# lighttransport/pbrlab

Measured on AMD Instinct MI355X. Metric: Msamples/s (paths x spp / s), 1920x1080 Cornell-box-Suzanne render, higher is better.
Workload: dtype f32

## Files before the change

pbrlab_amd/csrc/kernels.hip:

```cpp
#include <type_traits>

#include "dcamera.h"
#include "dshade.h"
#include "kernels.h"
#include "dtrace_pv.h"
#include "dtrace_quad.h"

namespace pb {

constexpr int kBlock = 256;

__device__ __forceinline__ uint32_t wave_sum(uint32_t v) {
#pragma unroll
  for (int o = 32; o > 0; o >>= 1) v += (uint32_t)__shfl_xor((int)v, o);
  return v;
}

__device__ __forceinline__ float4 mk4(V3 v, float w) { return make_float4(v.x, v.y, v.z, w); }

__device__ __forceinline__ void camera_sample(const PathState& P, uint32_t j, V3& dir, uint64_t& rng_state) {
  const uint32_t R = P.pass_run, q = j / R;
  const uint32_t pass = P.first_pass + (q / P.npix) * R + j % R;
  const uint32_t gpix = P.pix_index[q % P.npix];
  const uint32_t x = gpix % P.width, y = gpix / P.width;
// ... 442 lines not shown
      uint32_t i = tile * kTileItems + j * kBlock + threadIdx.x;
      e[j] = 0;
      if (i < n) e[j] = (i < n0) ? P.q_principled[i] : ((i < n0 + n1) ? P.q_hair[i - n0] : P.q_sss[i - n0 - n1]);
    }
    auto resumes = [](uint32_t w) { return (w & (kRAlive | kRResume)) == kRResume; };
    auto holds = [](uint32_t w) { return (w & (kRAlive | kRResume | kRHold)) == kRHold; };
    TileCompactor<2, kItemsPerThread> ta = {wcount, base, {}};
    {
      uint32_t dest[kItemsPerThread];
#pragma unroll
      for (int j = 0; j < kItemsPerThread; j++) dest[j] = ((e[j] & kRAlive) || resumes(e[j]) || holds(e[j])) ? 1u : 0u;
      ta.run(dest, counters);
#pragma unroll
      for (int j = 0; j < kItemsPerThread; j++)
        if (dest[j])
          P.q_out[ta.slot(j, 1u)] = resumes(e[j]) ? ((e[j] & (kRPathMask | kQDoomed)) | kQResume | ((e[j] & kRResumeFirst) ? kQFirst : 0u))
                                    : (holds(e[j]) ? ((e[j] & kRPathMask) | kQHold | ((e[j] & kRHoldDoomed) ? kQDoomed : 0u))
                                                   : (e[j] & (kRPathMask | kQSssBit | kQDoomed)));
      __syncthreads();
    }
    {
      uint32_t dest[kItemsPerThread];
#pragma unroll
      for (int j = 0; j < kItemsPerThread; j++) dest[j] = ((e[j] & kRShadow) && !resumes(e[j]) && !holds(e[j])) ? 2u : 0u;
      ta.run(dest, counters);
#pragma unroll
      for (int j = 0; j < kItemsPerThread; j++)
        if (dest[j]) P.q_shadow[ta.slot(j, 2u)] = e[j] & kRPathMask;
      __syncthreads();
    }
  }
}

struct PathHead {
  Hit h;
  V3 dir, thr;
  Surface s;
  Rng rng;
  uint32_t flags;
};
enum : int { kHeadEnds = 0, kHeadGoes = 1, kHeadHeld = 2 };
template <bool HOLD = true, bool ENV = false>
__device__ __forceinline__ int path_head(const PathState& P, const DScene& sc, uint32_t p, uint64_t rng_inc, PathHead& c, bool first) {
  float4 h4 = P.hit[p];
  float4 o4 = make_float4(P.cam_org[0], P.cam_org[1], P.cam_org[2], 0.0f), t4 = make_float4(1.0f, 1.0f, 1.0f, 0.0f);
  c.flags = first ? 0u : kFlagNotFirst;
  uint64_t rng_state;
  bool held = false;
  if (!first) {
    o4 = P.ray_o[p], t4 = P.thr[p];
    c.dir = ld3(P.ray_d[p]);
    if (HOLD) {
      const uint4 r4 = P.rng4[p];
      rng_state = (uint64_t)r4.x | ((uint64_t)r4.y << 32);
      held = P.no_medium != 0u && r4.z != 0u;
    } else {
      rng_state = P.rng[p];
    }
  } else {
    camera_sample(P, p - P.slot0, c.dir, rng_state);
  }
  c.h.t = h4.x, c.h.u = h4.y, c.h.v = h4.z, c.h.slot = __float_as_uint(h4.w);
  c.s = make_surface(sc, ld3(o4), c.dir, c.h);
  c.thr = ld3(t4);
  if (!held && c.s.face == kFront && c.s.lightrec != kNone) {
    const float4* lr = reinterpret_cast<const float4*>(sc.lrecs + c.s.lightrec);
    float pdf_area = lr[0].w;
    if (ENV) pdf_area = pdf_area * sc.env_area_scale;
    V3 emission = ld3(lr[4]);
    float a2s = fabsf((c.h.t * c.h.t) / dot(c.s.n_s, c.dir));
    float w = (c.flags & kFlagNotFirst) ? power_heuristic(t4.w, pdf_area * a2s) : 1.0f;
    float4 L4 = P.L[p];
    P.L[p] = mk4(ld3(L4) + w * emission * c.thr, L4.w);
  }
  c.rng.state = rng_state, c.rng.inc = rng_inc;
  float rr = spectrum_norm(c.thr);
  float u = draw(c.rng);
// ... 43 lines not shown
__device__ __forceinline__ bool misses_all_lights(const DScene& sc, V3 o, V3 d, float tmin) {
  if (sc.lights_transformed) return false;
  if (sc.num_lrecs <= kLightPretest) {
    const V3 inv(1.0f / d.x, 1.0f / d.y, 1.0f / d.z);
    for (uint32_t i = 0; i < sc.num_lrecs; i += 2u) {
      const float4* la = reinterpret_cast<const float4*>(sc.lrecs + i);
      const float4* lb = reinterpret_cast<const float4*>(sc.lrecs + (i + 1u < sc.num_lrecs ? i + 1u : i));
      const float4 a0 = la[0], a1 = la[1], a2 = la[2], b0 = lb[0], b1 = lb[1], b2 = lb[2];
      bool ok_a, ok_b;
      f2 t, u, v;
      tri_test_pair(make_float4(a0.x, b0.x, a0.y, b0.y), make_float4(a0.z, b0.z, a1.x, b1.x), make_float4(a1.y, b1.y, a1.z, b1.z),
                    make_float4(a2.x, b2.x, a2.y, b2.y), make_float4(a2.z, b2.z, 0.f, 0.f), o.x, o.y, o.z, d.x, d.y, d.z, inv.x, inv.y, inv.z, tmin, ok_a,
                    ok_b, t, u, v);
      if (ok_a || ok_b) return false;
    }
    return true;
  }
  if (sc.num_lights > kLightPretest) return false;
  const V3 inv(1.0f / d.x, 1.0f / d.y, 1.0f / d.z);
  for (uint32_t i = 0; i < (sc.num_lights + 1u) / 2u; i++) {
    const float4* np = reinterpret_cast<const float4*>(sc.light_boxes + i);
    bool h0, h1;
    float t0, t1;
    box_test2(np[0], np[1], np[2], o, inv, tmin, kInf, h0, h1, t0, t1);
    if (h0 || h1) return false;
  }
  return true;
}

__device__ __forceinline__ void count_pruned(const PathState& P) {
  if (P.stats) atomicAdd(&P.stats[kStatPrunedRays], 1ull);
}

__device__ __forceinline__ void put_shadow(const PathState& P, V3 pos, const Nee& n, V3 c_vis, V3 c_occ, uint32_t p,
                                           uint32_t mode, bool alive) {
  static_assert(kEps == 1e-3f, "shadow rays share (origin, tmin) with the continuation ray");
  if (!alive) P.ray_o[p] = mk4(pos, kEps);
  P.sh_d[p] = mk4(n.dir, smax(kEps, n.dist - kEps));
  P.sh_c[p] = mk4(c_vis, __uint_as_float(mode));
  if (mode == kShSssExit) P.sh_e[p] = mk4(c_occ, 0.f);
}

__device__ __forceinline__ bool stage_light_tables(const DScene& sc, float* lds) {
  if (!(sc.num_lights > 0 && sc.num_lights <= kLdsLights && sc.num_lrecs <= kLdsLights)) return false;
  constexpr uint32_t kRecWords = sizeof(LightRec) / 4;
  for (uint32_t i = threadIdx.x; i < sc.num_lights; i += kBlock) {
    lds[i] = sc.light_cdf[i];
    lds[kLdsLights + 2u * i] = __uint_as_float(sc.light_heads[i].first);
    lds[kLdsLights + 2u * i + 1u] = __uint_as_float(sc.light_heads[i].count);
  }
  for (uint32_t i = threadIdx.x; i < sc.num_lrecs; i += kBlock) lds[3u * kLdsLights + i] = sc.lprim_cdf[i];
  for (uint32_t i = threadIdx.x; i < sc.num_lrecs * kRecWords; i += kBlock) lds[4u * kLdsLights + i] = reinterpret_cast<const float*>(sc.lrecs)[i];
  return true;
}

enum : int { kShadePlain = 0, kShadeMedia = 1, kShadeFull = 2, kShadeEnv = 4 };
constexpr int shade_base(int mode) { return mode & 3; }
constexpr bool shade_env(int mode) { return (mode & kShadeEnv) != 0; }
template <int MODE_ = kShadeFull>
__device__ __forceinline__ uint32_t shade_principled_path(const PathState& P, const DScene& sc, uint32_t p, uint64_t rng_inc, bool first,
                                                          const PrincipledBsdf* lds_bsdf = nullptr, const float* lds_lights = nullptr) {
  constexpr int MODE = shade_base(MODE_);
  constexpr bool ENV = shade_env(MODE_);
  if (ENV && __float_as_uint(P.hit[p].w) == kNone) return env_miss_path<MODE != kShadeMedia>(P, sc, p, first);
  bool alive = false, shadow = false;
  V3 sh_pos(0.f), c_vis(0.f);
  Nee nee;
  nee.dir = V3(0.f), nee.emission = V3(0.f), nee.dist = 0.f, nee.pdf_sigma = 0.f;
  uint32_t sh_mode = kShNormal, qbit = 0u;
  PathHead c;
  const int head = path_head<MODE != kShadeMedia, ENV>(P, sc, p, rng_inc, c, first);
  if (head == kHeadGoes) {
    const Hit& h = c.h;
    const V3 dir = c.dir, thr = c.thr;
    const Surface& s = c.s;
    Rng& rng = c.rng;
    V3 new_thr(0.f), next_dir = -dir;
    float new_pdf = 0.f;
    if (s.face != kAmbiguous) {
      V3 wo_g = -dir;
      Frame fr;
      fr.ez = (s.face == kFront) ? s.n_s : -s.n_s;
      branchless_onb(fr.ez, fr.ex, fr.ey);
      V3 wo = to_local(fr, wo_g);
      PrincipledBsdf b;
      if (lds_bsdf) {
        constexpr uint32_t kWords = sizeof(PrincipledBsdf) / 4;
        const auto* lw = (const __attribute__((address_space(3))) uint32_t*)reinterpret_cast<const uint32_t*>(lds_bsdf) + s.material * kWords;
        uint32_t w[kWords];
#pragma unroll
        for (uint32_t k = 0; k < kWords; k++) w[k] = lw[k];
        __builtin_memcpy(&b, w, sizeof(b));
      } else {
        b = sc.materials[s.material].bsdf;
      }
      const bool per_hit = MODE == kShadeFull && sc.materials[s.material].textured != 0u;
      if (per_hit) {
        const PrincipledParam mp = sc.materials[s.material].param;
        V3 bc(mp.base_color[0], mp.base_color[1], mp.base_color[2]);
        V3 ssc(mp.subsurface_color[0], mp.subsurface_color[1], mp.subsurface_color[2]);
        if (mp.base_color_tex_id != kNone) bc = texture_fetch3(sc, mp.base_color_tex_id, s.tu, s.tv);
        if (mp.subsurface_color_tex_id != kNone) ssc = texture_fetch3(sc, mp.subsurface_color_tex_id, s.tu, s.tv);
        b = param_to_bsdf(mp, bc, ssc);
      }
// ... 23 lines not shown
      } else if (pick == 3) {
        float u0 = draw(rng);
        float u1 = draw(rng);
        ggx_sample(wo, b.clearcoat_alpha_x, b.clearcoat_alpha_y, u0, u1, wi);
      } else if (MODE == kShadePlain) {
        sampled = false;
      } else {
        sampled = false;
        bool ok = (s.face == kFront);
        if (ok) {
          float u0 = draw(rng);
          float u1 = draw(rng);
          V3 tmp;
          float pdf;
          lambert_sample(u0, u1, tmp, pdf);
          tmp = -tmp;
          V3 gdir = to_global(fr, tmp);
          ok = !(dot(-s.n_g, gdir) <= 0.0f);
          if (ok) {
            V3 sigt, sigs, wthr;
            if (per_hit) {
              medium_coefficients(b, sigt, sigs, wthr);
            } else {
              const float4* mc = reinterpret_cast<const float4*>(&sc.materials[s.material].sss_sigt);
              const float4 m0 = mc[0], m1 = mc[1], m2 = mc[2];
              sigt = V3(m0.x, m0.y, m0.z), sigs = V3(m0.w, m1.x, m1.y), wthr = V3(m1.z, m1.w, m2.x);
            }
            float e0 = draw(rng);
            float e1 = draw(rng);
            V3 chpdf;
            float t_scatter = sample_scatter_distance(wthr, sigs, sigt, e0, e1, chpdf);
            P.ray_o[p] = mk4(s.pos, 1e-3f);
            P.ray_d[p] = mk4(gdir, t_scatter);
            P.sss_sigt[p] = mk4(sigt, 0.f);
            P.sss_sigs[p] = mk4(sigs, __uint_as_float(sc.shade[h.slot & kHitSlotMask].instance_id));
            P.sss_thr[p] = mk4(wthr, __uint_as_float(0u));
            P.sss_ez[p] = mk4(fr.ez, 0.f);
            P.sss_A[p] = make_float4(0.f, 0.f, 0.f, 0.f);
            P.thr[p] = mk4(thr, 0.f);
            P.rng[p] = rng.state;
            alive = true;
            qbit = kQSssBit;
            sh_mode = kShSssEntry;
            c_vis = d1;
          }
        }
      }
      if (sampled) {
        V3 f;
        float pdf;
        eval_bsdf(wi, wo, b, w, f, pdf);
        next_dir = to_global(fr, wi);
        float cos_i = fabsf(wi.z);
        new_thr = f * cos_i / pdf;
        new_pdf = pdf;
        if (!is_finite(new_thr) || !isfinite(new_pdf)) {
          new_thr = V3(0.f);
          new_pdf = 0.f;
        }
      }
      if (sh_mode == kShNormal) c_vis = thr * ((V3(0.f) + d1) + V3(0.f));
      if (!alive) {
        V3 t2 = new_thr * thr;
        if (!is_black(t2)) {
          qbit = doomed_bit(t2, rng.state, rng_inc);
          if (!(qbit && !ENV && misses_all_lights(sc, s.pos, next_dir, 1e-3f))) {
            alive = true;
            P.ray_o[p] = mk4(s.pos, 1e-3f);
            P.ray_d[p] = mk4(next_dir, kInf);
            P.thr[p] = mk4(t2, new_pdf);
            store_rng<MODE != kShadeMedia>(P, p, rng.state);
          } else {
            qbit = 0u;
            count_pruned(P);
          }
        }
      }
    }
  }
  if (shadow) put_shadow(P, sh_pos, nee, c_vis, V3(0.f), p, sh_mode, alive);
  return head == kHeadHeld ? kRHold : ((shadow ? kRShadow : 0u) | (alive ? kRAlive : 0u) | qbit);
}
#ifndef PB_SHADE_WAVES
#define PB_SHADE_WAVES 4
#endif
#ifndef PB_LDS_MATS
#define PB_LDS_MATS 64
#endif
constexpr uint32_t kLdsMats = PB_LDS_MATS;
#ifndef PB_SHADE_WAVES_FULL
#define PB_SHADE_WAVES_FULL 3
#endif
#ifndef PB_SHADE_WAVES_MEDIA
#define PB_SHADE_WAVES_MEDIA 4
#endif
#ifndef PB_SHADE_WAVES_MEDIA_ENV
#define PB_SHADE_WAVES_MEDIA_ENV 3
#endif
constexpr int shade_waves(int mode) {
  return shade_base(mode) == kShadePlain ? PB_SHADE_WAVES
                                         : (shade_base(mode) == kShadeMedia ? (shade_env(mode) ? PB_SHADE_WAVES_MEDIA_ENV : PB_SHADE_WAVES_MEDIA) : PB_SHADE_WAVES_FULL);
}
template <int MODE_>
__global__ __launch_bounds__(kBlock, shade_waves(MODE_)) void k_shade_principled(PathState P, DScene sc, uint64_t rng_inc) {
  constexpr int MODE = shade_base(MODE_);
  constexpr bool ENV = shade_env(MODE_);
  __shared__ PrincipledBsdf lds_bsdf[kLdsMats ? kLdsMats : 1];
  __shared__ float lds_lights[kLdsMats ? kLdsLightWords : 1];
  const bool lights_staged = kLdsMats && stage_light_tables(sc, lds_lights);
  const bool staged = kLdsMats && sc.num_materials <= kLdsMats;
  if (staged) {
    constexpr uint32_t kWords = sizeof(PrincipledBsdf) / 4;
    static_assert(sizeof(PrincipledBsdf) % 4 == 0, "closure set is a whole number of words");
    uint32_t* dst = reinterpret_cast<uint32_t*>(lds_bsdf);
    for (uint32_t i = threadIdx.x; i < sc.num_materials * kWords; i += kBlock)
      dst[i] = reinterpret_cast<const uint32_t*>(&sc.materials[i / kWords].bsdf)[i % kWords];
  }
  if (staged || lights_staged) __syncthreads();
  const bool direct = P.direct != 0u;
  const uint32_t n = P.counts[direct ? kCntIn : kCntPrincipled];
  for (uint32_t i = blockIdx.x * kBlock + threadIdx.x; i < n; i += gridDim.x * kBlock) {
    constexpr bool kAnyBounce = MODE != kShadeMedia;
    const uint32_t e = direct ? ((!kAnyBounce || P.first) ? P.slot0 + i : P.q_in[i]) : P.q_principled[i];
    const uint32_t p = e & kQPathMask;
    uint32_t r = 0u;
    bool go = true;
    if (direct) {
      const uint32_t code = __float_as_uint(P.hit[p].w);
      const bool doomed = kAnyBounce && (e & kQDoomed);
      go = !(code == kNone || (!(code & kHitLight) && (doomed || (code & kHitNoMaterial))));
      if (ENV && code == kNone) go = true;
      if (code == kHitSuspended) {
        go = false, r = kRResume | kRResumeFirst;
        if (kAnyBounce && !P.first) r = kRResume | (e & kQDoomed) | ((e & kQFirst) ? kRResumeFirst : 0u);
      }
    } else if (e & kQResume) {
      go = false, r = kRResume | (e & kQDoomed) | ((e & kQFirst) ? kRResumeFirst : 0u);
    }
    if (go) r = shade_principled_path<MODE_>(P, sc, p, rng_inc, P.first != 0u || (e & kQFirst) != 0u, staged ? lds_bsdf : nullptr, lights_staged ? lds_lights : nullptr);
    if (r == kRHold && (e & kQDoomed) && (kAnyBounce ? !P.first : !direct)) r |= kRHoldDoomed;
    P.q_principled[i] = p | r;
  }
}

template <bool ENV = false>
__device__ __forceinline__ uint32_t shade_hair_path(const PathState& P, const DScene& sc, uint32_t p, uint64_t rng_inc, bool first,
                                                    const float* lds_lights = nullptr) {
  bool alive = false, shadow = false;
  uint32_t qbit = 0u;
  V3 sh_pos(0.f), c_vis(0.f);
  Nee nee;
  nee.dir = V3(0.f), nee.emission = V3(0.f), nee.dist = 0.f, nee.pdf_sigma = 0.f;
  PathHead c;
  const int head = path_head<true, ENV>(P, sc, p, rng_inc, c, first);
  if (head == kHeadGoes) {
    const Hit& h = c.h;
    const V3 dir = c.dir, thr = c.thr;
    const Surface& s = c.s;
    Rng& rng = c.rng;
    if (s.face != kAmbiguous) {
      V3 wo_g = -dir;
      Frame fr;
      fr.ex = s.n_s;
      fr.ey = vnormalize(cross(cross(wo_g, fr.ex), fr.ex));
      fr.ez = cross(fr.ex, fr.ey);
      V3 wo = to_local(fr, wo_g);
      HairBsdf hb = sc.materials[s.material].hair;
      hb.h = h.v;
      HairSetup S;
      hair_prepare(wo, hb, S);
      V3 d1(0.f);
      shadow = nee_sample<ENV>(sc, rng, s.pos, fr.ex, false, nee, lds_lights);
      if (shadow) {
        V3 wl = to_local(fr, nee.dir);
        float pdf;
        V3 fcos = hair_eval(S, wl, hb, pdf);
        d1 = nee_contribution(nee, fcos / fabsf(wl.x), pdf);
        sh_pos = s.pos;
      }
      float us[4];
      us[0] = draw(rng), us[1] = draw(rng), us[2] = draw(rng), us[3] = draw(rng);
      V3 wi(0.f);
      float pdf = 0.f;
      V3 fcos = hair_sample(S, hb, us, wi, pdf);
      V3 next_dir = to_global(fr, wi);
      V3 new_thr = fcos / pdf;
      if (!is_finite(new_thr) || !isfinite(pdf)) {
        new_thr = V3(0.f);
        pdf = 0.f;
      }
      c_vis = thr * ((V3(0.f) + d1) + V3(0.f));
      V3 t2 = new_thr * thr;
      if (!is_black(t2)) {
        qbit = doomed_bit(t2, rng.state, rng_inc);
        if (!(qbit && !ENV && misses_all_lights(sc, s.pos, next_dir, 1e-3f))) {
          alive = true;
          P.ray_o[p] = mk4(s.pos, 1e-3f);
          P.ray_d[p] = mk4(next_dir, kInf);
          P.thr[p] = mk4(t2, pdf);
          store_rng(P, p, rng.state);
        } else {
          qbit = 0u;
          count_pruned(P);
        }
      }
    }
  }
  if (shadow) put_shadow(P, sh_pos, nee, c_vis, V3(0.f), p, kShNormal, alive);
  return head == kHeadHeld ? kRHold : ((shadow ? kRShadow : 0u) | (alive ? kRAlive : 0u) | qbit);
}
template <bool ENV>
__global__ __launch_bounds__(kBlock) void k_shade_hair(PathState P, DScene sc, uint64_t rng_inc) {
  __shared__ float lds_lights[kLdsLightWords];
  const bool lights_staged = stage_light_tables(sc, lds_lights);
  if (lights_staged) __syncthreads();
  const uint32_t n = P.counts[kCntHair];
  for (uint32_t i = blockIdx.x * kBlock + threadIdx.x; i < n; i += gridDim.x * kBlock) {
    const uint32_t e = P.q_hair[i], p = e & kQPathMask;
    uint32_t r = shade_hair_path<ENV>(P, sc, p, rng_inc, P.first != 0u || (e & kQFirst) != 0u, lights_staged ? lds_lights : nullptr);
    if (r == kRHold && (e & kQDoomed)) r |= kRHoldDoomed;
    P.q_hair[i] = p | r;
  }
}

struct WalkState {
  V3 org, dir, sigt, sigs, wthr;
  float t_scatter;
  uint32_t bounce;
  uint64_t rng_state;
};
__device__ __forceinline__ bool sss_scatter(WalkState& w, uint64_t rng_inc, V3* chpdf_io = nullptr, bool have_chpdf = false, const V3* albedo = nullptr) {
  const V3 chpdf = (chpdf_io && have_chpdf) ? *chpdf_io : scatter_channel_pdf(w.wthr, w.sigs, w.sigt, albedo);
  const V3 trans = attenuate_transmission(w.sigt, w.t_scatter);
  float pdf = dot(chpdf, w.sigt * trans);
  V3 wthr = w.wthr * (w.sigs * trans) / pdf;
  float pr = saturate(spectrum_norm(wthr));
  Rng rng = {w.rng_state, rng_inc};
  float q = draw(rng);
  if (q >= pr) return false;
  wthr = wthr / pr;
  const V3 org = w.org + w.t_scatter * w.dir;
  const uint32_t bounce = w.bounce + 1u;
  if (bounce > 8192u) return false;
  float first = draw(rng);
  float second = draw(rng);
  V3 wi = vnormalize(uniform_sample_sphere(second, first));
  float e0 = draw(rng);
  float e1 = draw(rng);
  V3 chpdf_next;
  float t_scatter = sample_scatter_distance(wthr, w.sigs, w.sigt, e0, e1, chpdf_next, albedo);
  w.org = org, w.dir = wi, w.wthr = wthr, w.t_scatter = t_scatter, w.bounce = bounce, w.rng_state = rng.state;
  if (chpdf_io) *chpdf_io = chpdf_next;
  return true;
}

template <bool ENV = false>
__device__ __forceinline__ uint32_t sss_step_path(const PathState& P, const DScene& sc, uint32_t p, uint64_t rng_inc,
                                                  const Hit* hreg = nullptr, const float* lds_lights = nullptr) {
  bool alive = false, shadow = false;
  uint32_t qbit = 0u;
  V3 sh_pos(0.f), c_vis(0.f), c_occ(0.f);
  Nee nee;
  nee.dir = V3(0.f), nee.emission = V3(0.f), nee.dist = 0.f, nee.pdf_sigma = 0.f;
  float4 o4 = P.ray_o[p], d4 = P.ray_d[p];
  float4 st4 = P.sss_sigt[p], ss4 = P.sss_sigs[p], wt4 = P.sss_thr[p];
  Hit h;
  if (hreg) {
    h = *hreg;
  } else {
    const float4 h4 = P.hit[p];
    h.t = h4.x, h.u = h4.y, h.v = h4.z, h.slot = __float_as_uint(h4.w);
  }
  V3 org = ld3(o4), dir = ld3(d4), sigt = ld3(st4), sigs = ld3(ss4), wthr = ld3(wt4);
  uint32_t bounce = __float_as_uint(wt4.w), entry_inst = __float_as_uint(ss4.w);
  Rng rng = {P.rng[p], rng_inc};
  bool hit = (h.slot != kNone);
  bool fail = false, exited = false;
  if (hit) {
    V3 chpdf = scatter_channel_pdf(wthr, sigs, sigt);
    V3 trans = attenuate_transmission(sigt, h.t);
    float pdf = dot(chpdf, trans);
    wthr = wthr * trans / pdf;
    exited = true;
  } else {
    WalkState w = {org, dir, sigt, sigs, wthr, d4.w , bounce, rng.state};
    if (!sss_scatter(w, rng_inc)) {
      fail = true;
    } else {
      P.ray_o[p] = mk4(w.org, 0.f);
      P.ray_d[p] = mk4(w.dir, w.t_scatter);
      P.sss_thr[p] = mk4(w.wthr, __uint_as_float(w.bounce));
      P.rng[p] = w.rng_state;
      alive = true;
      qbit = kQSssBit;
    }
  }
  V3 thr = ld3(P.thr[p]);
  V3 A = ld3(P.sss_A[p]);
  if (alive) {
  } else if (exited) {
    uint32_t exit_inst;
    Surface s = make_surface(sc, org, dir, h, &exit_inst);
    if (exit_inst != entry_inst) fail = true;
    if (s.face != kBack) fail = true;
    if (!fail) {
      Frame fx;
      fx.ez = s.n_s;
      branchless_onb(fx.ez, fx.ex, fx.ey);
      V3 wo = to_local(fx, dir);
      PrincipledBsdf nb = default_bsdf();
      nb.enable_diffuse = 1;
      nb.diffuse_weight = wthr;
      SampleWeight w = closure_sample_weight(wo, nb);
      V3 d2(0.f);
      shadow = nee_sample<ENV>(sc, rng, s.pos, s.n_s, true, nee, lds_lights);
      if (shadow) {
        V3 f;
        float pdf;
        eval_bsdf(to_local(fx, nee.dir), wo, nb, w, f, pdf);
        d2 = nee_contribution(nee, f, pdf);
        sh_pos = s.pos;
      }
      float select = draw(rng);
// ... 2 lines not shown
      float u0 = draw(rng);
      float u1 = draw(rng);
      if (pick == 0) {
        float pdf;
        lambert_sample(u0, u1, wi, pdf);
      } else {
        ggx_sample(wo, nb.clearcoat_alpha_x, nb.clearcoat_alpha_y, u0, u1, wi);
      }
      V3 f;
      float pdf;
      eval_bsdf(wi, wo, nb, w, f, pdf);
      Frame fe;
      fe.ez = ld3(P.sss_ez[p]);
      branchless_onb(fe.ez, fe.ex, fe.ey);
      V3 next_dir = to_global(fe, wi);
      V3 new_thr = f * fabsf(wi.z) / pdf;
      if (!is_finite(new_thr) || !isfinite(pdf)) {
        new_thr = V3(0.f);
        pdf = 0.f;
      }
      c_vis = thr * (A + d2);
      c_occ = thr * (A + V3(0.f));
      if (!shadow) {
        float4 L4 = P.L[p];
        P.L[p] = mk4(ld3(L4) + c_occ, L4.w);
      }
      V3 t2 = new_thr * thr;
      if (!is_black(t2)) {
        qbit = doomed_bit(t2, rng.state, rng_inc);
        if (!(qbit && !ENV && misses_all_lights(sc, s.pos, next_dir, 1e-3f))) {
          alive = true;
          P.ray_o[p] = mk4(s.pos, 1e-3f);
          P.ray_d[p] = mk4(next_dir, kInf);
          P.thr[p] = mk4(t2, pdf);
          P.rng[p] = rng.state;
        } else {
          qbit = 0u;
          count_pruned(P);
        }
      }
    }
  }
  if (fail) {
    float4 L4 = P.L[p];
    P.L[p] = mk4(ld3(L4) + thr * (A + V3(0.f)), L4.w);
  }
  if (shadow) put_shadow(P, sh_pos, nee, c_vis, c_occ, p, kShSssExit, alive);
  return (shadow ? kRShadow : 0u) | (alive ? kRAlive : 0u) | qbit;
}
template <bool ENV>
__global__ __launch_bounds__(kBlock) void k_sss_step(PathState P, DScene sc, uint64_t rng_inc) {
  __shared__ float lds_lights[kLdsLightWords];
  const bool lights_staged = stage_light_tables(sc, lds_lights);
  if (lights_staged) __syncthreads();
  const uint32_t n = P.counts[kCntSss];
  for (uint32_t i = blockIdx.x * kBlock + threadIdx.x; i < n; i += gridDim.x * kBlock) {
    const uint32_t p = P.q_sss[i];
    P.q_sss[i] = p | sss_step_path<ENV>(P, sc, p, rng_inc, nullptr, lights_staged ? lds_lights : nullptr);
  }
}

#ifndef PB_WALK_CAP
#define PB_WALK_CAP 24u
#endif
constexpr uint32_t kWalkCap = PB_WALK_CAP;
constexpr uint32_t kWalkWords = 22;
struct WalkSink {
  static constexpr bool kWalk = true, kSplit = false, kSuspend = false;
  const PathState& P;
  uint64_t rng_inc;
  float* wl;
  uint32_t n_rays;
  __device__ __forceinline__ void start(uint32_t idx, uint32_t& tag, Hit& h, V3& o, V3& d) {
    tag = idx;
    const uint32_t p = P.q_sss[idx] & kQPathMask;
    const float4 h4 = P.hit[p];
    h.t = h4.x, h.u = h4.y, h.v = h4.z, h.slot = __float_as_uint(h4.w);
    wl[7 * kBlock] = __uint_as_float(0u), wl[8 * kBlock] = __uint_as_float(p);
    wl[21 * kBlock] = __uint_as_float(kNone);
    if (h.slot == kNone) {
// ... 79 lines not shown
};
#ifndef PB_WALK_WAVES
#define PB_WALK_WAVES 3
#endif
#ifndef PB_WALK_WAVES_TRI
#define PB_WALK_WAVES_TRI 4
#endif
constexpr uint32_t walk_blocks_per_cu(bool curves, bool wide) { return (!curves && wide) ? PB_WALK_WAVES_TRI : PB_WALK_WAVES; }
template <bool STATS, bool CURVES, bool WIDE = false>
__global__ __launch_bounds__(kBlock, STATS ? PB_WALK_WAVES : walk_blocks_per_cu(CURVES, WIDE)) void k_sss_walk(PathState P, DScene sc, uint64_t rng_inc) {
  __shared__ uint32_t stk[pv_lds_stack<CURVES, WIDE>() * kBlock];
  __shared__ float frm[CURVES ? 10 * kBlock : 1];
  __shared__ float walk[kWalkWords * kBlock];
  const uint32_t n = P.counts[kCntSss];
  TravStats st = {};
  uint32_t overflow = 0u;
  WalkSink sink = {P, rng_inc, walk + threadIdx.x, 0u};
  trace_pv<0, STATS, CURVES, WIDE>(sc, n, &P.counts[kCntWalkHead], sink, stk + threadIdx.x, kBlock,
                             P.spill + blockIdx.x * kBlock + threadIdx.x, gridDim.x * kBlock, st, &overflow,
                             CURVES ? frm + threadIdx.x : nullptr);
  if (overflow) P.counts[kCntOverflow] = 1u;
  if (STATS) {
    const uint32_t a = wave_sum(sink.n_rays), nn = wave_sum(st.nodes), nt = wave_sum(st.tris + st.curves);
    if (__lane_id() == 0 && a) atomicAdd(&P.stats[kStatTailClosestRays], (unsigned long long)a);
    if (__lane_id() == 0) {
      atomicAdd(&P.stats[kStatWalkNodes], (unsigned long long)nn), atomicAdd(&P.stats[kStatWalkTris], (unsigned long long)nt);
      atomicAdd(&P.stats[kStatWalkTurns], (unsigned long long)(st.it_node + st.it_tri + st.it_curve));
      atomicAdd(&P.stats[kStatWalkSteps], (unsigned long long)st.it_refill);
      atomicAdd(&P.stats[kStatWalkCycTrav], st.cyc[0] + st.cyc[1] + st.cyc[2]), atomicAdd(&P.stats[kStatWalkCycStep], st.cyc[3]);
    }
  }
}

#ifndef PB_TAIL_OCTETS
#define PB_TAIL_OCTETS 1
#endif
#ifndef PB_TAIL_WAVES
#define PB_TAIL_WAVES 3
#endif
template <int MODE_, bool STATS, bool CURVES, bool WIDE = false>
__global__ __launch_bounds__(kBlock, PB_TAIL_WAVES) void k_tail(PathState P, DScene sc, uint64_t rng_inc) {
  constexpr int MODE = shade_base(MODE_);
  constexpr bool ENV = shade_env(MODE_);
  __shared__ uint32_t stk[kSimpleLdsStack * kBlock];
  uint32_t* const spill = P.spill + blockIdx.x * kBlock + threadIdx.x;
  const uint32_t spill_stride = gridDim.x * kBlock;
  const uint32_t n = P.counts[kCntIn];
  const uint32_t lane = threadIdx.x & 63u;
  const uint32_t wave = (blockIdx.x * kBlock + threadIdx.x) >> 6, nwaves = gridDim.x * (kBlock >> 6);
  uint32_t per_wave = (n + nwaves - 1u) / nwaves;
  per_wave = per_wave < 1u ? 1u : (per_wave > 64u ? 64u : per_wave);
  TravStats st = {};
  uint32_t overflow = 0u, n_closest = 0u, n_shadow = 0u;
  const TraceSink sink = {P, 0u, 0u};
  uint32_t* const stack = stk + threadIdx.x;
  constexpr uint32_t kHave = 0x80000000u, kMedium = 0x40000000u, kFirst = 0x20000000u;
  constexpr bool kOctets = PB_TAIL_OCTETS != 0 && WIDE && !CURVES;
  for (uint32_t base = wave * per_wave; base < n; base += nwaves * per_wave) {
    uint32_t state = 0u;
    if (lane < per_wave && base + lane < n) {
      const uint32_t e = P.first ? P.slot0 + base + lane : P.q_in[base + lane];
      state = (e & kQPathMask) | kHave | ((!P.no_medium && (e & kQSssBit)) ? kMedium : 0u) | ((P.first || (e & kQFirst)) ? kFirst : 0u);
    }
    uint32_t team = 1u;
    for (;;) {
      const unsigned long long act = __ballot((state & kHave) != 0u);
      if (act == 0ull) break;
      const uint32_t alive = (uint32_t)__popcll(act);
      const uint32_t want_team = (kOctets && alive <= 8u) ? 8u : (alive <= 32u ? 2u : 1u);
      if (want_team > team) {
        uint32_t src = lane;
        bool mine = false;
        uint32_t k = 0;
        for (unsigned long long m = act; m; m &= m - 1ull, k++)
          if (lane == want_team * k) src = (uint32_t)__builtin_ctzll(m), mine = true;
        const uint32_t moved = (uint32_t)__shfl((int)state, (int)src);
        state = mine ? moved : 0u;
        team = want_team;
      }
      const bool paired = team == 2u;
      const uint32_t p = state & kQPathMask;
      uint32_t r = 0u;
      if (state & kHave) {
        if (MODE != kShadePlain && (state & kMedium)) {
          r = sss_step_path<ENV>(P, sc, p, rng_inc);
        } else {
          const uint32_t slot = __float_as_uint(P.hit[p].w);
          if (slot != kNone)
            r = (slot & kHitHair) ? shade_hair_path<ENV>(P, sc, p, rng_inc, (state & kFirst) != 0u)
                                  : shade_principled_path<MODE_>(P, sc, p, rng_inc, (state & kFirst) != 0u);
          else if (ENV)
            r = env_miss_path<MODE != kShadeMedia>(P, sc, p, (state & kFirst) != 0u);
        }
        state &= ~kFirst;
      }
      const bool want_shadow = (r & kRShadow) != 0u, want_closest = (r & kRAlive) != 0u;
      if (kOctets && team == 8u) {
        const bool upper = (lane & 4u) != 0u;
        float4 o4 = make_float4(0.f, 0.f, 0.f, 0.f), d4 = o4, s4 = o4;
        if (want_shadow || want_closest) o4 = P.ray_o[p];
        if (want_closest) d4 = P.ray_d[p];
        if (want_shadow) s4 = P.sh_d[p];
        const int lead = (int)(lane & ~7u);
        const float ox = __shfl(o4.x, lead), oy = __shfl(o4.y, lead), oz = __shfl(o4.z, lead), ow = __shfl(o4.w, lead);
        const float cx = __shfl(d4.x, lead), cy = __shfl(d4.y, lead), cz = __shfl(d4.z, lead), cw = __shfl(d4.w, lead);
        const float sx = __shfl(s4.x, lead), sy = __shfl(s4.y, lead), sz = __shfl(s4.z, lead), sw = __shfl(s4.w, lead);
        const float dx = upper ? sx : cx, dy = upper ? sy : cy, dz = upper ? sz : cz, dw = upper ? sw : cw;
        const uint32_t wants = (uint32_t)__shfl((int)((want_closest ? 1u : 0u) | (want_shadow ? 2u : 0u)), lead);
        const bool go = (wants & (upper ? 2u : 1u)) != 0u;
        Hit h = {0.f, 0.f, 0.f, kNone};
        bool occluded = false;
        const uint32_t col = threadIdx.x & ~3u;
        if (go) occluded = traverse_quad<2>(sc, V3(ox, oy, oz), V3(dx, dy, dz), ow, dw, h, stk + col, kBlock, &overflow, upper,
                                            P.spill + blockIdx.x * kBlock + col, spill_stride);
        const bool occ_up = __shfl((int)occluded, lead + 4) != 0;
        if (want_shadow) {
          Hit none = {0.f, 0.f, 0.f, kNone};
          sink.done(p | 0x80000000u, none, occ_up);
          n_shadow++;
        }
        if (want_closest) {
          P.hit[p] = make_float4(h.t, h.u, h.v, __uint_as_float(h.slot));
          n_closest++;
        }
      } else if (!paired) {
        if (want_shadow) {
          const float4 o4 = P.ray_o[p], d4 = P.sh_d[p];
          Hit h;
          const bool occluded = traverse<true, false, CURVES, WIDE>(sc, ld3(o4), ld3(d4), o4.w, d4.w, h, stack, kBlock, st, &overflow, spill, spill_stride);
          sink.done(p | 0x80000000u, h, occluded);
          n_shadow++;
        }
        if (want_closest) {
          const float4 o4 = P.ray_o[p], d4 = P.ray_d[p];
          Hit h;
          traverse<false, false, CURVES, WIDE>(sc, ld3(o4), ld3(d4), o4.w, d4.w, h, stack, kBlock, st, &overflow, spill, spill_stride);
          P.hit[p] = make_float4(h.t, h.u, h.v, __uint_as_float(h.slot));
          n_closest++;
        }
      } else {
        const bool odd = (lane & 1u) != 0u;
        float4 o4 = make_float4(0.f, 0.f, 0.f, 0.f), d4 = o4, s4 = o4;
        if (want_shadow || want_closest) o4 = P.ray_o[p];
        if (want_closest) d4 = P.ray_d[p];
        if (want_shadow) s4 = P.sh_d[p];
        const int left = (int)(lane & ~1u);
        const float sx = __shfl(s4.x, left), sy = __shfl(s4.y, left), sz = __shfl(s4.z, left), sw = __shfl(s4.w, left);
        const float ox = __shfl(o4.x, left), oy = __shfl(o4.y, left), oz = __shfl(o4.z, left), ow = __shfl(o4.w, left);
        const bool left_shadow = __shfl((int)want_shadow, left) != 0;
        bool go = want_closest;
        if (odd) o4 = make_float4(ox, oy, oz, ow), d4 = make_float4(sx, sy, sz, sw), go = left_shadow;
        Hit h = {0.f, 0.f, 0.f, kNone};
        bool occluded = false;
        if (go) occluded = traverse_mode<2, false, CURVES, WIDE>(sc, ld3(o4), ld3(d4), o4.w, d4.w, h, stack, kBlock, st, &overflow, odd, spill, spill_stride);
        const bool occ_right = __shfl((int)occluded, (int)(lane | 1u)) != 0;
        if (want_shadow) {
          Hit none = {0.f, 0.f, 0.f, kNone};
          sink.done(p | 0x80000000u, none, occ_right);
          n_shadow++;
        }
        if (want_closest) {
          P.hit[p] = make_float4(h.t, h.u, h.v, __uint_as_float(h.slot));
          n_closest++;
        }
      }
      if (!want_closest) state = 0u;
      else state = (state & ~kMedium) | ((r & kQSssBit) ? kMedium : 0u);
    }
  }
  if (overflow) P.counts[kCntOverflow] = 1u;
  if (STATS) {
    const uint32_t a = wave_sum(n_closest), b = wave_sum(n_shadow);
    if (lane == 0 && a) atomicAdd(&P.stats[kStatTailClosestRays], (unsigned long long)a);
    if (lane == 0 && b) atomicAdd(&P.stats[kStatTailShadowRays], (unsigned long long)b);
  }
}

__global__ __launch_bounds__(kBlock) void k_accumulate(PathState P, const uint32_t* __restrict__ pix_index, uint32_t npix,
                                                       uint32_t npass, float* __restrict__ rgba,
                                                       uint32_t* __restrict__ count) {
  const uint32_t R = P.pass_run;
  for (uint32_t i = blockIdx.x * kBlock + threadIdx.x; i < npix; i += gridDim.x * kBlock) {
    uint32_t g = pix_index[i];
    float4 acc = reinterpret_cast<float4*>(rgba)[g];
    uint32_t c = count[g];
    if (R == 1u) {
      for (uint32_t k = 0; k < npass; k++) {
        float4 L = P.L[(size_t)k * npix + i];
        acc.x += L.x, acc.y += L.y, acc.z += L.z, acc.w += 1.0f;
        c++;
      }
    } else {
      for (uint32_t k0 = 0; k0 < npass; k0 += R) {
        const float4* run = P.L + ((size_t)(k0 / R) * npix + i) * R;
        for (uint32_t r0 = 0; r0 < R; r0 += 8u) {
          float4 L[8];
#pragma unroll
          for (uint32_t r = 0; r < 8u; r++) L[r] = (r0 + r < R) ? run[r0 + r] : make_float4(0.f, 0.f, 0.f, 0.f);
// ... 432 lines not shown
```

Baseline: 3126.

## Carry hits and rays in registers through the tail kernel and stage LDS tables

The tail megakernel now keeps each lane's hit record in registers, shuffles it along with state during team regrouping, and hands the freshly written ray origin, direction and shadow data from shading straight to traversal. This avoids re-reading values from global memory that were just written. It also stages material BSDFs and light tables into LDS for the tail kernel, and replaces the trace sink with an inline shadow-delivery routine that can use the carried shadow colour and radiance. In exchange the kernel uses more registers and LDS, which can lower occupancy, and it adds several compile-time mode predicates.

After: 3126. Within noise of the previous version (-0.0%).

```diff
diff --git a/pbrlab_amd/csrc/kernels.hip b/pbrlab_amd/csrc/kernels.hip
--- a/pbrlab_amd/csrc/kernels.hip
+++ b/pbrlab_amd/csrc/kernels.hip
@@ -498,6 +498,9 @@
   }
 }
 
+struct TailHand {
+  float4 ray_o, ray_d, sh_d, sh_c;
+};
 struct PathHead {
   Hit h;
   V3 dir, thr;
@@ -506,9 +509,12 @@
   uint32_t flags;
 };
 enum : int { kHeadEnds = 0, kHeadGoes = 1, kHeadHeld = 2 };
-template <bool HOLD = true, bool ENV = false>
-__device__ __forceinline__ int path_head(const PathState& P, const DScene& sc, uint32_t p, uint64_t rng_inc, PathHead& c, bool first) {
-  float4 h4 = P.hit[p];
+template <bool HOLD = true, bool ENV = false, bool TAIL = false>
+__device__ __forceinline__ int path_head(const PathState& P, const DScene& sc, uint32_t p, uint64_t rng_inc, PathHead& c, bool first,
+                                         const Hit* hin = nullptr) {
+  float4 h4;
+  if constexpr (TAIL) h4 = make_float4(hin->t, hin->u, hin->v, __uint_as_float(hin->slot));
+  else h4 = P.hit[p];
   float4 o4 = make_float4(P.cam_org[0], P.cam_org[1], P.cam_org[2], 0.0f), t4 = make_float4(1.0f, 1.0f, 1.0f, 0.0f);
   c.flags = first ? 0u : kFlagNotFirst;
   uint64_t rng_state;
@@ -618,13 +624,19 @@
   if (P.stats) atomicAdd(&P.stats[kStatPrunedRays], 1ull);
 }
 
+template <bool TAIL = false>
 __device__ __forceinline__ void put_shadow(const PathState& P, V3 pos, const Nee& n, V3 c_vis, V3 c_occ, uint32_t p,
-                                           uint32_t mode, bool alive) {
+                                           uint32_t mode, bool alive, TailHand* out = nullptr) {
   static_assert(kEps == 1e-3f, "shadow rays share (origin, tmin) with the continuation ray");
   if (!alive) P.ray_o[p] = mk4(pos, kEps);
   P.sh_d[p] = mk4(n.dir, smax(kEps, n.dist - kEps));
   P.sh_c[p] = mk4(c_vis, __uint_as_float(mode));
   if (mode == kShSssExit) P.sh_e[p] = mk4(c_occ, 0.f);
+  if constexpr (TAIL) {
+    if (!alive) out->ray_o = mk4(pos, kEps);
+    out->sh_d = mk4(n.dir, smax(kEps, n.dist - kEps));
+    out->sh_c = mk4(c_vis, __uint_as_float(mode));
+  }
 }
 
 __device__ __forceinline__ bool stage_light_tables(const DScene& sc, float* lds) {
@@ -643,19 +655,20 @@
 enum : int { kShadePlain = 0, kShadeMedia = 1, kShadeFull = 2, kShadeEnv = 4 };
 constexpr int shade_base(int mode) { return mode & 3; }
 constexpr bool shade_env(int mode) { return (mode & kShadeEnv) != 0; }
-template <int MODE_ = kShadeFull>
+template <int MODE_ = kShadeFull, bool TAIL = false>
 __device__ __forceinline__ uint32_t shade_principled_path(const PathState& P, const DScene& sc, uint32_t p, uint64_t rng_inc, bool first,
-                                                          const PrincipledBsdf* lds_bsdf = nullptr, const float* lds_lights = nullptr) {
+                                                          const PrincipledBsdf* lds_bsdf = nullptr, const float* lds_lights = nullptr,
+                                                          TailHand* out = nullptr, const Hit* hin = nullptr) {
   constexpr int MODE = shade_base(MODE_);
   constexpr bool ENV = shade_env(MODE_);
-  if (ENV && __float_as_uint(P.hit[p].w) == kNone) return env_miss_path<MODE != kShadeMedia>(P, sc, p, first);
+  if (!TAIL && ENV && __float_as_uint(P.hit[p].w) == kNone) return env_miss_path<MODE != kShadeMedia>(P, sc, p, first);
   bool alive = false, shadow = false;
   V3 sh_pos(0.f), c_vis(0.f);
   Nee nee;
   nee.dir = V3(0.f), nee.emission = V3(0.f), nee.dist = 0.f, nee.pdf_sigma = 0.f;
   uint32_t sh_mode = kShNormal, qbit = 0u;
   PathHead c;
-  const int head = path_head<MODE != kShadeMedia, ENV>(P, sc, p, rng_inc, c, first);
+  const int head = path_head<MODE != kShadeMedia, ENV, TAIL>(P, sc, p, rng_inc, c, first, hin);
   if (head == kHeadGoes) {
     const Hit& h = c.h;
     const V3 dir = c.dir, thr = c.thr;
@@ -745,6 +758,7 @@
             float t_scatter = sample_scatter_distance(wthr, sigs, sigt, e0, e1, chpdf);
             P.ray_o[p] = mk4(s.pos, 1e-3f);
             P.ray_d[p] = mk4(gdir, t_scatter);
+            if constexpr (TAIL) out->ray_o = mk4(s.pos, 1e-3f), out->ray_d = mk4(gdir, t_scatter);
             P.sss_sigt[p] = mk4(sigt, 0.f);
             P.sss_sigs[p] = mk4(sigs, __uint_as_float(sc.shade[h.slot & kHitSlotMask].instance_id));
             P.sss_thr[p] = mk4(wthr, __uint_as_float(0u));
@@ -781,6 +795,7 @@
             alive = true;
             P.ray_o[p] = mk4(s.pos, 1e-3f);
             P.ray_d[p] = mk4(next_dir, kInf);
+            if constexpr (TAIL) out->ray_o = mk4(s.pos, 1e-3f), out->ray_d = mk4(next_dir, kInf);
             P.thr[p] = mk4(t2, new_pdf);
             store_rng<MODE != kShadeMedia>(P, p, rng.state);
           } else {
@@ -791,7 +806,7 @@
       }
     }
   }
-  if (shadow) put_shadow(P, sh_pos, nee, c_vis, V3(0.f), p, sh_mode, alive);
+  if (shadow) put_shadow<TAIL>(P, sh_pos, nee, c_vis, V3(0.f), p, sh_mode, alive, out);
   return head == kHeadHeld ? kRHold : ((shadow ? kRShadow : 0u) | (alive ? kRAlive : 0u) | qbit);
 }
 #ifndef PB_SHADE_WAVES
@@ -856,16 +871,16 @@
   }
 }
 
-template <bool ENV = false>
+template <bool ENV = false, bool TAIL = false>
 __device__ __forceinline__ uint32_t shade_hair_path(const PathState& P, const DScene& sc, uint32_t p, uint64_t rng_inc, bool first,
-                                                    const float* lds_lights = nullptr) {
+                                                    const float* lds_lights = nullptr, TailHand* out = nullptr, const Hit* hin = nullptr) {
   bool alive = false, shadow = false;
   uint32_t qbit = 0u;
   V3 sh_pos(0.f), c_vis(0.f);
   Nee nee;
   nee.dir = V3(0.f), nee.emission = V3(0.f), nee.dist = 0.f, nee.pdf_sigma = 0.f;
   PathHead c;
-  const int head = path_head<true, ENV>(P, sc, p, rng_inc, c, first);
+  const int head = path_head<true, ENV, TAIL>(P, sc, p, rng_inc, c, first, hin);
   if (head == kHeadGoes) {
     const Hit& h = c.h;
     const V3 dir = c.dir, thr = c.thr;
@@ -910,6 +925,7 @@
           alive = true;
           P.ray_o[p] = mk4(s.pos, 1e-3f);
           P.ray_d[p] = mk4(next_dir, kInf);
+          if constexpr (TAIL) out->ray_o = mk4(s.pos, 1e-3f), out->ray_d = mk4(next_dir, kInf);
           P.thr[p] = mk4(t2, pdf);
           store_rng(P, p, rng.state);
         } else {
@@ -919,7 +935,7 @@
       }
     }
   }
-  if (shadow) put_shadow(P, sh_pos, nee, c_vis, V3(0.f), p, kShNormal, alive);
+  if (shadow) put_shadow<TAIL>(P, sh_pos, nee, c_vis, V3(0.f), p, kShNormal, alive, out);
   return head == kHeadHeld ? kRHold : ((shadow ? kRShadow : 0u) | (alive ? kRAlive : 0u) | qbit);
 }
 template <bool ENV>
@@ -967,9 +983,9 @@
   return true;
 }
 
-template <bool ENV = false>
+template <bool ENV = false, bool TAIL = false>
 __device__ __forceinline__ uint32_t sss_step_path(const PathState& P, const DScene& sc, uint32_t p, uint64_t rng_inc,
-                                                  const Hit* hreg = nullptr, const float* lds_lights = nullptr) {
+                                                  const Hit* hreg = nullptr, const float* lds_lights = nullptr, TailHand* out = nullptr) {
   bool alive = false, shadow = false;
   uint32_t qbit = 0u;
   V3 sh_pos(0.f), c_vis(0.f), c_occ(0.f);
@@ -1002,6 +1018,7 @@
     } else {
       P.ray_o[p] = mk4(w.org, 0.f);
       P.ray_d[p] = mk4(w.dir, w.t_scatter);
+      if constexpr (TAIL) out->ray_o = mk4(w.org, 0.f), out->ray_d = mk4(w.dir, w.t_scatter);
       P.sss_thr[p] = mk4(w.wthr, __uint_as_float(w.bounce));
       P.rng[p] = w.rng_state;
       alive = true;
@@ -1070,6 +1087,7 @@
           alive = true;
           P.ray_o[p] = mk4(s.pos, 1e-3f);
           P.ray_d[p] = mk4(next_dir, kInf);
+          if constexpr (TAIL) out->ray_o = mk4(s.pos, 1e-3f), out->ray_d = mk4(next_dir, kInf);
           P.thr[p] = mk4(t2, pdf);
           P.rng[p] = rng.state;
         } else {
@@ -1083,7 +1101,7 @@
     float4 L4 = P.L[p];
     P.L[p] = mk4(ld3(L4) + thr * (A + V3(0.f)), L4.w);
   }
-  if (shadow) put_shadow(P, sh_pos, nee, c_vis, c_occ, p, kShSssExit, alive);
+  if (shadow) put_shadow<TAIL>(P, sh_pos, nee, c_vis, c_occ, p, kShSssExit, alive, out);
   return (shadow ? kRShadow : 0u) | (alive ? kRAlive : 0u) | qbit;
 }
 template <bool ENV>
@@ -1229,17 +1247,53 @@
   }
 }
 
+template <bool CARRIED>
+__device__ __forceinline__ void tail_deliver(const PathState& P, uint32_t p, float4 c, float4 L, bool occluded) {
+  if (occluded && P.no_medium) return;
+  if (!CARRIED) c = P.sh_c[p], L = P.L[p];
+  const uint32_t mode = __float_as_uint(c.w);
+  if (mode == kShSssEntry) {
+    if (!occluded) P.sss_A[p] = make_float4(0.0f + c.x, 0.0f + c.y, 0.0f + c.z, 0.0f);
+  } else if (!occluded || mode == kShSssExit) {
+    V3 add(c.x, c.y, c.z);
+    if (occluded) add = ld3(P.sh_e[p]);
+    P.L[p] = make_float4(L.x + add.x, L.y + add.y, L.z + add.z, L.w);
+  }
+}
 #ifndef PB_TAIL_OCTETS
 #define PB_TAIL_OCTETS 1
 #endif
 #ifndef PB_TAIL_WAVES
 #define PB_TAIL_WAVES 3
 #endif
+constexpr bool tail_octets(bool curves, bool wide) { return PB_TAIL_OCTETS != 0 && wide && !curves; }
+constexpr bool tail_hands_over(int mode, bool stats, bool curves, bool wide) {
+  if (tail_octets(curves, wide)) return mode == kShadePlain;
+  return !(stats && curves && wide && mode == kShadeFull);
+}
+constexpr bool tail_carries(int mode, bool stats, bool curves, bool wide) { return tail_hands_over(mode, stats, curves, wide) && !tail_octets(curves, wide); }
+constexpr bool tail_stages_bsdf(int mode, bool curves, bool wide) { return kLdsMats != 0 && !(tail_octets(curves, wide) && mode == (kShadeFull | kShadeEnv)); }
+constexpr bool tail_stages_lights(int mode, bool stats, bool curves, bool wide) { return !(stats && tail_octets(curves, wide) && mode == (kShadeFull | kShadeEnv)); }
 template <int MODE_, bool STATS, bool CURVES, bool WIDE = false>
 __global__ __launch_bounds__(kBlock, PB_TAIL_WAVES) void k_tail(PathState P, DScene sc, uint64_t rng_inc) {
   constexpr int MODE = shade_base(MODE_);
   constexpr bool ENV = shade_env(MODE_);
   __shared__ uint32_t stk[kSimpleLdsStack * kBlock];
+  constexpr bool kStageBsdf = tail_stages_bsdf(MODE_, CURVES, WIDE);
+  __shared__ PrincipledBsdf lds_bsdf[kStageBsdf ? kLdsMats : 1];
+  constexpr bool kStageLights = tail_stages_lights(MODE_, STATS, CURVES, WIDE);
+  __shared__ float lds_lights[kStageLights ? kLdsLightWords : 1];
+  const bool lights_staged = kStageLights && stage_light_tables(sc, lds_lights);
+  const bool staged = kStageBsdf && sc.num_materials <= kLdsMats;
+  if (staged) {
+    constexpr uint32_t kWords = sizeof(PrincipledBsdf) / 4;
+    uint32_t* dst = reinterpret_cast<uint32_t*>(lds_bsdf);
+    for (uint32_t i = threadIdx.x; i < sc.num_materials * kWords; i += kBlock)
+      dst[i] = reinterpret_cast<const uint32_t*>(&sc.materials[i / kWords].bsdf)[i % kWords];
+  }
+  if (staged || lights_staged) __syncthreads();
+  const PrincipledBsdf* const bsdf_tab = staged ? lds_bsdf : nullptr;
+  const float* const light_tab = lights_staged ? lds_lights : nullptr;
   uint32_t* const spill = P.spill + blockIdx.x * kBlock + threadIdx.x;
   const uint32_t spill_stride = gridDim.x * kBlock;
   const uint32_t n = P.counts[kCntIn];
@@ -1249,15 +1303,18 @@
   per_wave = per_wave < 1u ? 1u : (per_wave > 64u ? 64u : per_wave);
   TravStats st = {};
   uint32_t overflow = 0u, n_closest = 0u, n_shadow = 0u;
-  const TraceSink sink = {P, 0u, 0u};
   uint32_t* const stack = stk + threadIdx.x;
   constexpr uint32_t kHave = 0x80000000u, kMedium = 0x40000000u, kFirst = 0x20000000u;
-  constexpr bool kOctets = PB_TAIL_OCTETS != 0 && WIDE && !CURVES;
+  constexpr bool kOctets = tail_octets(CURVES, WIDE);
+  constexpr bool kHand = tail_hands_over(MODE_, STATS, CURVES, WIDE), kCarry = tail_carries(MODE_, STATS, CURVES, WIDE);
   for (uint32_t base = wave * per_wave; base < n; base += nwaves * per_wave) {
     uint32_t state = 0u;
+    Hit hit = {0.f, 0.f, 0.f, kNone};
     if (lane < per_wave && base + lane < n) {
       const uint32_t e = P.first ? P.slot0 + base + lane : P.q_in[base + lane];
       state = (e & kQPathMask) | kHave | ((!P.no_medium && (e & kQSssBit)) ? kMedium : 0u) | ((P.first || (e & kQFirst)) ? kFirst : 0u);
+      const float4 h4 = P.hit[e & kQPathMask];
+      hit.t = h4.x, hit.u = h4.y, hit.v = h4.z, hit.slot = __float_as_uint(h4.w);
     }
     uint32_t team = 1u;
     for (;;) {
@@ -1273,31 +1330,41 @@
           if (lane == want_team * k) src = (uint32_t)__builtin_ctzll(m), mine = true;
         const uint32_t moved = (uint32_t)__shfl((int)state, (int)src);
         state = mine ? moved : 0u;
+        hit.t = __shfl(hit.t, (int)src), hit.u = __shfl(hit.u, (int)src), hit.v = __shfl(hit.v, (int)src);
+        hit.slot = (uint32_t)__shfl((int)hit.slot, (int)src);
         team = want_team;
       }
       const bool paired = team == 2u;
       const uint32_t p = state & kQPathMask;
       uint32_t r = 0u;
+      if (!kHand && (state & kHave)) hit.slot = __float_as_uint(P.hit[p].w);
+      const float4 zero4 = make_float4(0.f, 0.f, 0.f, 0.f);
+      const float any = __builtin_nondeterministic_value(0.f);
+      const float4 any4 = make_float4(any, any, any, any);
+      TailHand hand = {any4, any4, any4, any4};
       if (state & kHave) {
         if (MODE != kShadePlain && (state & kMedium)) {
-          r = sss_step_path<ENV>(P, sc, p, rng_inc);
+          r = sss_step_path<ENV, kHand>(P, sc, p, rng_inc, kHand ? &hit : nullptr, light_tab, &hand);
         } else {
-          const uint32_t slot = __float_as_uint(P.hit[p].w);
+          const uint32_t slot = hit.slot;
           if (slot != kNone)
-            r = (slot & kHitHair) ? shade_hair_path<ENV>(P, sc, p, rng_inc, (state & kFirst) != 0u)
-                                  : shade_principled_path<MODE_>(P, sc, p, rng_inc, (state & kFirst) != 0u);
+            r = (slot & kHitHair) ? shade_hair_path<ENV, kHand>(P, sc, p, rng_inc, (state & kFirst) != 0u, light_tab, &hand, &hit)
+                                  : shade_principled_path<MODE_, kHand>(P, sc, p, rng_inc, (state & kFirst) != 0u, bsdf_tab, light_tab, &hand, &hit);
           else if (ENV)
             r = env_miss_path<MODE != kShadeMedia>(P, sc, p, (state & kFirst) != 0u);
         }
         state &= ~kFirst;
       }
       const bool want_shadow = (r & kRShadow) != 0u, want_closest = (r & kRAlive) != 0u;
+      float4 L4 = zero4;
+      if (kCarry && want_shadow) L4 = P.L[p];
+      Hit h = {0.f, 0.f, 0.f, kNone};
       if (kOctets && team == 8u) {
         const bool upper = (lane & 4u) != 0u;
-        float4 o4 = make_float4(0.f, 0.f, 0.f, 0.f), d4 = o4, s4 = o4;
-        if (want_shadow || want_closest) o4 = P.ray_o[p];
-        if (want_closest) d4 = P.ray_d[p];
-        if (want_shadow) s4 = P.sh_d[p];
+        float4 o4 = zero4, d4 = zero4, s4 = zero4;
+        if (want_shadow || want_closest) o4 = kHand ? hand.ray_o : P.ray_o[p];
+        if (want_closest) d4 = kHand ? hand.ray_d : P.ray_d[p];
+        if (want_shadow) s4 = kHand ? hand.sh_d : P.sh_d[p];
         const int lead = (int)(lane & ~7u);
         const float ox = __shfl(o4.x, lead), oy = __shfl(o4.y, lead), oz = __shfl(o4.z, lead), ow = __shfl(o4.w, lead);
         const float cx = __shfl(d4.x, lead), cy = __shfl(d4.y, lead), cz = __shfl(d4.z, lead), cw = __shfl(d4.w, lead);
@@ -1305,15 +1372,13 @@
         const float dx = upper ? sx : cx, dy = upper ? sy : cy, dz = upper ? sz : cz, dw = upper ? sw : cw;
         const uint32_t wants = (uint32_t)__shfl((int)((want_closest ? 1u : 0u) | (want_shadow ? 2u : 0u)), lead);
         const bool go = (wants & (upper ? 2u : 1u)) != 0u;
-        Hit h = {0.f, 0.f, 0.f, kNone};
         bool occluded = false;
         const uint32_t col = threadIdx.x & ~3u;
         if (go) occluded = traverse_quad<2>(sc, V3(ox, oy, oz), V3(dx, dy, dz), ow, dw, h, stk + col, kBlock, &overflow, upper,
                                             P.spill + blockIdx.x * kBlock + col, spill_stride);
         const bool occ_up = __shfl((int)occluded, lead + 4) != 0;
         if (want_shadow) {
-          Hit none = {0.f, 0.f, 0.f, kNone};
-          sink.done(p | 0x80000000u, none, occ_up);
+          tail_deliver<kCarry>(P, p, hand.sh_c, L4, occ_up);
           n_shadow++;
         }
         if (want_closest) {
@@ -1322,38 +1387,35 @@
         }
       } else if (!paired) {
         if (want_shadow) {
-          const float4 o4 = P.ray_o[p], d4 = P.sh_d[p];
-          Hit h;
-          const bool occluded = traverse<true, false, CURVES, WIDE>(sc, ld3(o4), ld3(d4), o4.w, d4.w, h, stack, kBlock, st, &overflow, spill, spill_stride);
-          sink.done(p | 0x80000000u, h, occluded);
+          const float4 o4 = kHand ? hand.ray_o : P.ray_o[p], d4 = kHand ? hand.sh_d : P.sh_d[p];
+          Hit hs;
+          const bool occluded = traverse<true, false, CURVES, WIDE>(sc, ld3(o4), ld3(d4), o4.w, d4.w, hs, stack, kBlock, st, &overflow, spill, spill_stride);
+          tail_deliver<kCarry>(P, p, hand.sh_c, L4, occluded);
           n_shadow++;
         }
         if (want_closest) {
-          const float4 o4 = P.ray_o[p], d4 = P.ray_d[p];
-          Hit h;
+          const float4 o4 = kHand ? hand.ray_o : P.ray_o[p], d4 = kHand ? hand.ray_d : P.ray_d[p];
           traverse<false, false, CURVES, WIDE>(sc, ld3(o4), ld3(d4), o4.w, d4.w, h, stack, kBlock, st, &overflow, spill, spill_stride);
           P.hit[p] = make_float4(h.t, h.u, h.v, __uint_as_float(h.slot));
           n_closest++;
         }
       } else {
         const bool odd = (lane & 1u) != 0u;
-        float4 o4 = make_float4(0.f, 0.f, 0.f, 0.f), d4 = o4, s4 = o4;
-        if (want_shadow || want_closest) o4 = P.ray_o[p];
-        if (want_closest) d4 = P.ray_d[p];
-        if (want_shadow) s4 = P.sh_d[p];
+        float4 o4 = zero4, d4 = zero4, s4 = zero4;
+        if (want_shadow || want_closest) o4 = kHand ? hand.ray_o : P.ray_o[p];
+        if (want_closest) d4 = kHand ? hand.ray_d : P.ray_d[p];
+        if (want_shadow) s4 = kHand ? hand.sh_d : P.sh_d[p];
         const int left = (int)(lane & ~1u);
         const float sx = __shfl(s4.x, left), sy = __shfl(s4.y, left), sz = __shfl(s4.z, left), sw = __shfl(s4.w, left);
         const float ox = __shfl(o4.x, left), oy = __shfl(o4.y, left), oz = __shfl(o4.z, left), ow = __shfl(o4.w, left);
         const bool left_shadow = __shfl((int)want_shadow, left) != 0;
         bool go = want_closest;
         if (odd) o4 = make_float4(ox, oy, oz, ow), d4 = make_float4(sx, sy, sz, sw), go = left_shadow;
-        Hit h = {0.f, 0.f, 0.f, kNone};
         bool occluded = false;
         if (go) occluded = traverse_mode<2, false, CURVES, WIDE>(sc, ld3(o4), ld3(d4), o4.w, d4.w, h, stack, kBlock, st, &overflow, odd, spill, spill_stride);
         const bool occ_right = __shfl((int)occluded, (int)(lane | 1u)) != 0;
         if (want_shadow) {
-          Hit none = {0.f, 0.f, 0.f, kNone};
-          sink.done(p | 0x80000000u, none, occ_right);
+          tail_deliver<kCarry>(P, p, hand.sh_c, L4, occ_right);
           n_shadow++;
         }
         if (want_closest) {
@@ -1361,6 +1423,7 @@
           n_closest++;
         }
       }
+      hit = h;
       if (!want_closest) state = 0u;
       else state = (state & ~kMedium) | ((r & kQSssBit) ? kMedium : 0u);
     }
```
